# XuanchenLi/Topo4D

Hardware: AMD Instinct MI355X
Metric: rasterizer fwd+bwd views/sec (higher is better)
Workload: dtype f32

## Files before the change

### topo4d_amd/csrc/t4d_raster.hip

```cpp
#include <hip/hip_runtime.h>
#include <stdint.h>
#include <stdio.h>
#include <stdlib.h>
#include <string.h>
#include <vector>

#include "../../include/t4d_config.h"
#include "../../include/topo4d_raster.h"
#include "t4d_activations.h"

#define T4D_EXPORT extern "C" __attribute__((visibility("default")))

namespace {

constexpr int kBlock = 256;
#ifndef T4D_FWD_BATCH
#define T4D_FWD_BATCH 192
#endif
constexpr int kFwdBatch = T4D_FWD_BATCH;
#ifndef T4D_BWD_BATCH
#define T4D_BWD_BATCH 128
#endif
constexpr int kBwdBatch = T4D_BWD_BATCH;
constexpr int kSortLdsCap = 2048;
constexpr int kLongBlock = 1024;
constexpr int kScanChunk = 1024;
constexpr int kRankSortMax = 512;
constexpr int kHist = 1024;
constexpr int kBuckets = 24;
constexpr int kGP = T4D_GRAD_PAIR_FLOATS;
constexpr int kCursorSegs = 64;
#ifndef T4D_SEG
#define T4D_SEG 128
#endif
constexpr int kSeg = T4D_SEG;
constexpr int kSegOne = 64;
constexpr int kSegMaxTiles = 8192;
#ifndef T4D_SEG_LONG_MIN
#define T4D_SEG_LONG_MIN 2048
#endif
constexpr int kSegLongMin = T4D_SEG_LONG_MIN;
constexpr int kSnapFloats = 6;
static_assert((kSegLongMin & (kSegLongMin - 1)) == 0, "k_fwd_long_prefix stops at the first work item of a shorter length CLASS (powers of two)");

thread_local char g_err[512] = "";

enum KernelId { K_PREPROCESS = 0, K_SCAN_TILES, K_SCATTER, K_SORT_TILES, K_RENDER_FWD, K_RENDER_BWD, K_PREPROCESS_BWD,
                K_SORT_LONG, K_FWD_LONG, K_RENDER_BWD_LONG, K_COUNT };
const char *const kKernelNames[K_COUNT] = { "k_preprocess", "k_scan_tiles", "k_scatter", "k_sort_tiles", "k_render_fwd",
                                            "k_render_bwd", "k_preprocess_bwd", "k_sort_long", "k_fwd_long", "k_render_bwd_long" };
struct ProfRec { int id; hipEvent_t a, b; };
bool g_prof_on = false;
std::vector<ProfRec> g_prof;

struct Layout {
    size_t status, view_total, view_cursor, tile_count, bucket_fill, slot_tab, zero_end;
    size_t snap, live;
    size_t tile_off, chunk_sum, order, items, xy, depth, conic_opacity, rgb, clamped, pair_off, pair_rank, keys, sort_tmp, final_T, n_contrib, total;
};

struct DevStatus {
    uint32_t overflow;
    uint32_t max_pairs;
    unsigned long long total_pairs;
    uint32_t max_tile_pairs;
    uint32_t grid_sync;
    uint32_t live_segments;
};

inline size_t align_up(size_t x, size_t a = 256) { return (x + a - 1) / a * a; }

inline int seg_mode(const T4DProblem &p)
{
    const long long T = (long long)((p.W + T4D_TILE_X - 1) / T4D_TILE_X) * (long long)((p.H + T4D_TILE_Y - 1) / T4D_TILE_Y);
    if ((long long)p.n_views * T <= kSegMaxTiles) return 1;
    return p.n_views == 1 ? 2 : 0;
}
inline bool seg_capable(const T4DProblem &p) { return seg_mode(p) != 0; }
inline int seg_positions(const T4DProblem &p) { return (p.n_views == 1 && seg_mode(p) == 1) ? kSegOne : kSeg; }
inline size_t seg_slots_per_view(const T4DProblem &p, size_t T)
{
    if (seg_mode(p) == 2) return (size_t)p.pair_capacity / (size_t)kSeg + (size_t)p.pair_capacity / (size_t)kSegLongMin + 2;
    return (size_t)p.pair_capacity / (size_t)seg_positions(p) + T + 1;
}

Layout make_layout(const T4DProblem &p)
{
    Layout L;
    const size_t V = (size_t)p.n_views, P = (size_t)p.P;
    const size_t T = (size_t)((p.W + T4D_TILE_X - 1) / T4D_TILE_X) * (size_t)((p.H + T4D_TILE_Y - 1) / T4D_TILE_Y);
    const size_t HW = (size_t)p.H * p.W;
    const size_t cap = (size_t)p.pair_capacity;
    size_t o = 0;
    L.status = o;        o = align_up(o + sizeof(DevStatus));
    L.view_total = o;    o = align_up(o + V * 4);
    L.view_cursor = o;   o = align_up(o + V * kCursorSegs * 4);
    L.tile_count = o;    o = align_up(o + V * T * 4);
    L.bucket_fill = o;   o = align_up(o + kBuckets * 4);
    const size_t slots = seg_capable(p) ? V * seg_slots_per_view(p, T) : 0;
    L.slot_tab = o;      o = align_up(o + slots * 16);
    L.zero_end = o;
    L.snap = o;          o = align_up(o + slots * kSnapFloats * kBlock * 4);
    L.live = o;          o = align_up(o + (seg_mode(p) == 2 ? slots * 4 : 0));
    L.tile_off = o;      o = align_up(o + V * T * 4);
    L.chunk_sum = o;     o = align_up(o + V * ((T + kScanChunk - 1) / kScanChunk) * 4);
    L.order = o;         o = align_up(o + (size_t)kBuckets * V * T * 4);
    L.items = o;         o = align_up(o + V * T * 16);
    L.xy = o;            o = align_up(o + V * P * 8);
    L.depth = o;         o = align_up(o + V * P * 4);
    L.conic_opacity = o; o = align_up(o + V * P * 16);
    L.rgb = o;           o = align_up(o + (p.sh_coeffs > 0 ? V * P * 12 : 0));
    L.clamped = o;       o = align_up(o + (p.sh_coeffs > 0 ? V * P : 0));
    L.pair_off = o;      o = align_up(o + V * P * 4);
    L.pair_rank = o;     o = align_up(o + V * cap * 4);
    L.keys = o;          o = align_up(o + V * cap * 8);
    L.sort_tmp = o;      o = align_up(o + V * cap * 8);
    L.final_T = o;       o = align_up(o + V * HW * 4);
    L.n_contrib = o;     o = align_up(o + V * HW * 4);
    L.total = o;
    return L;
}

struct KP {
    int V, P, H, W, gx, gy, T, deg, M;
    float scale_modifier;
    uint32_t cap;
    uint32_t nseg, seg_cap;
    uint32_t seg_shift;
    const float *views, *means3D, *opacities, *scales, *rotations, *cov3D_precomp, *colors_precomp, *shs;
    DevStatus *status;
    uint32_t *view_total, *view_cursor, *tile_count, *bucket_fill, *tile_off, *chunk_sum, *order, *pair_off, *pair_rank;
    int n_chunks;
    int long_bins_elsewhere;
    int raw_params;
    uint4 *items;
    float2 *xy;
    float *depth;
    float4 *conic_opacity;
    float *rgb;
    uint8_t *clamped;
    unsigned long long *keys, *sort_tmp;
    float *cut_r2;
    float *final_T;
    uint32_t *n_contrib;
    float *out_color, *out_depth, *out_alpha;
    int32_t *radii;
    const float *dL_dcolor, *dL_ddepth, *dL_dalpha;
    float *grad_pair;
    float *dL_dmeans3D, *dL_dmeans2D, *dL_dcolors, *dL_dshs, *dL_dopacities, *dL_dscales, *dL_drotations, *dL_dcov3D;
    float *tile_dot;
    float *cotangent_dot;
    uint32_t tile_blocks;
    uint32_t fill_blocks;
    uint32_t fill_vec;
    uint4 *slot_tab;
    float *snap;
    uint32_t slots_per_view;
    uint32_t fused_sort;
    unsigned long long *host_status;
    uint32_t seg_min_pairs;
    uint32_t *live;
    uint32_t slots_by_offset;
    uint32_t views_per_set;
};

__device__ __forceinline__ float ndc2pix(float v, int S)
{
#pragma clang fp contract(off)
    return ((v + 1.0f) * S - 1.0f) * 0.5f;
}

__device__ __forceinline__ void tile_rect(float px, float py, int r, int gx, int gy, int &x0, int &y0, int &x1, int &y1)
{
    x0 = min(gx, max(0, (int)((px - r) / T4D_TILE_X)));
    y0 = min(gy, max(0, (int)((py - r) / T4D_TILE_Y)));
    x1 = min(gx, max(0, (int)((px + r + T4D_TILE_X - 1) / T4D_TILE_X)));
    y1 = min(gy, max(0, (int)((py + r + T4D_TILE_Y - 1) / T4D_TILE_Y)));
}

typedef const __attribute__((address_space(4))) float *const_float_p;
struct ViewRecord {
    float view[16], proj[16], campos[3], bg[3], tanx, tany;
};
__device__ __forceinline__ ViewRecord load_view_record(const float *views, const int v)
{
    const_float_p p = (const_float_p)(views + (size_t)v * T4D_VIEW_FLOATS);
    ViewRecord r;
#pragma unroll
    for (int i = 0; i < 16; i++) { r.view[i] = p[i]; r.proj[i] = p[16 + i]; }
#pragma unroll
    for (int i = 0; i < 3; i++) { r.campos[i] = p[32 + i]; r.bg[i] = p[35 + i]; }
    r.tanx = p[38]; r.tany = p[39];
    return r;
}

__device__ __forceinline__ size_t param_row0(const KP &kp, const int v)
{
    return kp.views_per_set ? (size_t)((uint32_t)v / kp.views_per_set) * (size_t)kp.P : (size_t)0;
}

__device__ __forceinline__ uint32_t seg_slot0(const KP &kp, const uint32_t off, const uint32_t tile)
{
    static_assert((kSegLongMin & (kSegLongMin - 1)) == 0, "a shift");
    return (off >> kp.seg_shift) + (kp.slots_by_offset ? off / (uint32_t)kSegLongMin : tile);
}

__device__ __forceinline__ uint32_t wave_incl_scan(uint32_t v)
{
    const int lane = threadIdx.x & 63;
#pragma unroll
    for (int d = 1; d < 64; d <<= 1) {
        uint32_t o = __shfl_up(v, d, 64);
        if (lane >= d) v += o;
    }
    return v;
}

template <int CTRL, int ROW_MASK = 0xf, int BANK_MASK = 0xf>
__device__ __forceinline__ float dpp0(float v)
{
    return __int_as_float(__builtin_amdgcn_update_dpp(0, __float_as_int(v), CTRL, ROW_MASK, BANK_MASK, false));
}

__device__ __forceinline__ float wave_sum_to_lane63(float v)
{
    v += dpp0<0xB1>(v);
    v += dpp0<0x4E>(v);
    v += dpp0<0x141>(v);
    v += dpp0<0x140>(v);
    v += dpp0<0x142, 0xA>(v);
    v += dpp0<0x143, 0xC>(v);
    return v;
}

__device__ __forceinline__ void quat_rot(const float4 q, float R[9])
{
#pragma clang fp contract(off)
    const float r = q.x, x = q.y, y = q.z, z = q.w;
    R[0] = 1.f - 2.f * (y * y + z * z); R[1] = 2.f * (x * y - r * z);       R[2] = 2.f * (x * z + r * y);
    R[3] = 2.f * (x * y + r * z);       R[4] = 1.f - 2.f * (x * x + z * z); R[5] = 2.f * (y * z - r * x);
    R[6] = 2.f * (x * z - r * y);       R[7] = 2.f * (y * z + r * x);       R[8] = 1.f - 2.f * (x * x + y * y);
}

__device__ __forceinline__ void cov3d_from_scale_rot(const float *scale, float mod, const float4 q, float cov[6])
{
#pragma clang fp contract(off)
// ... 149 lines not shown
        if (debug) {                                                                           \
            e_ = hipStreamSynchronize(stream);                                                 \
            if (e_ != hipSuccess) return fail(T4D_ERR_HIP, name " exec: %s", hipGetErrorString(e_)); \
        }                                                                                      \
    } while (0)

int device_cus()
{
    static int cus = 0;
    if (cus == 0) {
        int dev = 0, n = 0;
        if (hipGetDevice(&dev) != hipSuccess || hipDeviceGetAttribute(&n, hipDeviceAttributeMultiprocessorCount, dev) != hipSuccess || n <= 0)
            n = 256;
        cus = n;
    }
    return cus;
}

int tile_grid(int n_tiles, int per_cu, int div)
{
    static int env_div = -1;
    if (env_div < 0) {
        const char *d = getenv("T4D_TILE_DIV");
        env_div = d ? atoi(d) : 0;
    }
    if (env_div > 0) return max(min(n_tiles, device_cus() * per_cu), (n_tiles + env_div - 1) / env_div);
    constexpr int kMaxGridPerCu = 96;
    return max(min(n_tiles, device_cus() * per_cu), min((n_tiles + div - 1) / div, device_cus() * kMaxGridPerCu));
}

bool latency_launch(int n_tiles)
{
    const char *e = getenv("T4D_LATENCY_TILES");
    return n_tiles <= (e ? atoi(e) : 4 * device_cus());
}
bool latency_launch_fwd(int n_tiles, uint32_t flags)
{
    const char *e = getenv("T4D_FWD_LATENCY_TILES");
    if (!e) e = getenv("T4D_LATENCY_TILES");
    return n_tiles <= (e ? atoi(e) : ((flags & T4D_FLAG_LONG_LISTS) ? 24 : 12) * device_cus());
}

int check_problem(const T4DProblem *p)
{
    if (!p) return fail(T4D_ERR_ARG, "null problem");
    if (p->abi_version != T4D_ABI_VERSION) return fail(T4D_ERR_ARG, "abi_version mismatch");
    if (p->n_views < 1 || p->P < 1 || p->H < 1 || p->W < 1) return fail(T4D_ERR_ARG, "n_views, P, H, W must be >= 1");
    if (p->n_views > 4095) return fail(T4D_ERR_ARG, "n_views must be <= 4095");
    if ((int64_t)((p->W + T4D_TILE_X - 1) / T4D_TILE_X) * ((p->H + T4D_TILE_Y - 1) / T4D_TILE_Y) > 0xfffff)
        return fail(T4D_ERR_ARG, "image too large: more than 2^20 tiles");
    if ((int64_t)p->n_views * ((p->W + T4D_TILE_X - 1) / T4D_TILE_X) * ((p->H + T4D_TILE_Y - 1) / T4D_TILE_Y) > (1LL << 30))
        return fail(T4D_ERR_ARG, "n_views * tiles exceeds 2^30 work items: split the batch");
    if (p->pair_capacity < 1 || p->pair_capacity > 0x7fffffffLL) return fail(T4D_ERR_ARG, "pair_capacity out of range");
    if (p->views_per_param_set != 0u && (p->views_per_param_set > (uint32_t)p->n_views || (uint32_t)p->n_views % p->views_per_param_set != 0u))
        return fail(T4D_ERR_ARG, "n_views must be a multiple of views_per_param_set");
    if (p->sh_coeffs < 0 || p->sh_degree < 0 || p->sh_degree > 3) return fail(T4D_ERR_ARG, "sh_degree must be 0..3");
    if (p->sh_coeffs > 0 && p->sh_coeffs < (p->sh_degree + 1) * (p->sh_degree + 1))
        return fail(T4D_ERR_ARG, "sh_coeffs smaller than (sh_degree+1)^2");
    return T4D_OK;
}

void fill_common(KP &kp, const T4DProblem &p, const Layout &L, char *st)
{
    kp.V = p.n_views; kp.P = p.P; kp.H = p.H; kp.W = p.W;
    kp.gx = (p.W + T4D_TILE_X - 1) / T4D_TILE_X;
    kp.gy = (p.H + T4D_TILE_Y - 1) / T4D_TILE_Y;
    kp.T = kp.gx * kp.gy;
    kp.deg = p.sh_degree; kp.M = p.sh_coeffs;
    kp.scale_modifier = p.scale_modifier;
    kp.raw_params = (p.flags & T4D_FLAG_RAW_PARAMS) ? 1 : 0;
    kp.views_per_set = (p.views_per_param_set != 0u && p.views_per_param_set < (uint32_t)p.n_views) ? p.views_per_param_set : 0u;
    kp.cap = (uint32_t)p.pair_capacity;
    {
        const uint32_t n_wg = (uint32_t)((p.P + kBlock - 1) / kBlock);
        kp.nseg = 1;
        while (kp.nseg < (uint32_t)kCursorSegs && n_wg >= 16u * kp.nseg) kp.nseg <<= 1;
        kp.seg_cap = kp.cap / kp.nseg;
    }
    kp.status = reinterpret_cast<DevStatus *>(st + L.status);
    kp.view_total = reinterpret_cast<uint32_t *>(st + L.view_total);
    kp.view_cursor = reinterpret_cast<uint32_t *>(st + L.view_cursor);
    kp.tile_count = reinterpret_cast<uint32_t *>(st + L.tile_count);
    kp.bucket_fill = reinterpret_cast<uint32_t *>(st + L.bucket_fill);
    kp.order = reinterpret_cast<uint32_t *>(st + L.order);
    kp.items = reinterpret_cast<uint4 *>(st + L.items);
    kp.pair_rank = reinterpret_cast<uint32_t *>(st + L.pair_rank);
    kp.cut_r2 = reinterpret_cast<float *>(st + L.pair_rank);
    kp.tile_off = reinterpret_cast<uint32_t *>(st + L.tile_off);
    kp.chunk_sum = reinterpret_cast<uint32_t *>(st + L.chunk_sum);
    kp.n_chunks = (kp.T + kScanChunk - 1) / kScanChunk;
    kp.long_bins_elsewhere = (p.flags & T4D_FLAG_NO_LONG_BINS) ? 0 : 1;
    kp.pair_off = reinterpret_cast<uint32_t *>(st + L.pair_off);
    kp.xy = reinterpret_cast<float2 *>(st + L.xy);
    kp.depth = reinterpret_cast<float *>(st + L.depth);
    kp.conic_opacity = reinterpret_cast<float4 *>(st + L.conic_opacity);
    kp.rgb = reinterpret_cast<float *>(st + L.rgb);
    kp.clamped = reinterpret_cast<uint8_t *>(st + L.clamped);
    kp.keys = reinterpret_cast<unsigned long long *>(st + L.keys);
    kp.sort_tmp = reinterpret_cast<unsigned long long *>(st + L.sort_tmp);
    kp.final_T = reinterpret_cast<float *>(st + L.final_T);
    kp.n_contrib = reinterpret_cast<uint32_t *>(st + L.n_contrib);
    kp.slot_tab = reinterpret_cast<uint4 *>(st + L.slot_tab);
    kp.snap = reinterpret_cast<float *>(st + L.snap);
    kp.live = reinterpret_cast<uint32_t *>(st + L.live);
    kp.slots_per_view = seg_capable(p) ? (uint32_t)seg_slots_per_view(p, (size_t)kp.T) : 0u;
    kp.seg_shift = seg_positions(p) == 64 ? 6u : 7u;
    kp.slots_by_offset = seg_mode(p) == 2 ? 1u : 0u;
    kp.seg_min_pairs = seg_mode(p) == 2 ? ((p.flags & T4D_FLAG_NO_LONG_BINS) ? 0xffffffffu : (uint32_t)kSegLongMin) : 0u;
    static_assert(kSegOne == 64 && kSeg == 128, "seg_shift assumes segment lengths of 64 and 128");
}

}

T4D_EXPORT uint32_t t4d_abi_version(void) { return T4D_ABI_VERSION; }
T4D_EXPORT const char *t4d_last_error(void) { return g_err; }

T4D_EXPORT size_t t4d_state_bytes(const T4DProblem *prob)
{
    if (check_problem(prob) != T4D_OK) return 0;
    return make_layout(*prob).total;
}

size_t grad_pair_bytes(const T4DProblem &p) { return align_up((size_t)p.n_views * (size_t)p.pair_capacity * kGP * sizeof(float)); }
size_t tile_dot_bytes(const T4DProblem &p, size_t n_tiles) { return align_up((size_t)p.n_views * n_tiles * 4 * sizeof(float)); }

T4D_EXPORT size_t t4d_backward_scratch_bytes(const T4DProblem *prob)
{
    if (check_problem(prob) != T4D_OK) return 0;
    const size_t n_tiles = (size_t)((prob->W + T4D_TILE_X - 1) / T4D_TILE_X) * ((prob->H + T4D_TILE_Y - 1) / T4D_TILE_Y);
    return grad_pair_bytes(*prob) + tile_dot_bytes(*prob, n_tiles) +
           (prob->sh_coeffs > 0 ? align_up((size_t)prob->n_views * (size_t)prob->P * 3 * sizeof(float)) : 0);
}

T4D_EXPORT int t4d_debug_state_layout(const T4DProblem *prob, int has_sh, uint64_t *offsets, int n)
{
    int rc = check_problem(prob);
    if (rc != T4D_OK) return rc;
    if (!offsets || n < T4D_DEBUG_LAYOUT_FIELDS) return fail(T4D_ERR_ARG, "offsets must hold T4D_DEBUG_LAYOUT_FIELDS entries");
    T4DProblem p = *prob;
    if (!has_sh) p.sh_coeffs = 0;
    const Layout L = make_layout(p);
    const size_t f[T4D_DEBUG_LAYOUT_FIELDS] = { L.status, L.view_total, L.view_cursor, L.tile_count, L.bucket_fill, L.tile_off,
                                                L.xy, L.depth, L.conic_opacity, L.rgb, L.clamped, L.pair_off, L.keys,
                                                L.final_T, L.n_contrib, L.total };
    for (int i = 0; i < T4D_DEBUG_LAYOUT_FIELDS; i++) offsets[i] = (uint64_t)f[i];
    return T4D_OK;
}

static unsigned front_small_resident_blocks()
{
    static int cached_dev = -1;
    static unsigned cached = 0;
    int dev = 0;
    if (hipGetDevice(&dev) != hipSuccess) { (void)hipGetLastError(); return 0; }
    if (dev != cached_dev) {
        int per_cu = 0, cus = 0;
        if (hipOccupancyMaxActiveBlocksPerMultiprocessor(&per_cu, k_front_small, kBlock, 0) != hipSuccess ||
            hipDeviceGetAttribute(&cus, hipDeviceAttributeMultiprocessorCount, dev) != hipSuccess || per_cu < 1 || cus < 1) {
            (void)hipGetLastError();
            per_cu = 0; cus = 0;
        }
        cached = (unsigned)per_cu * (unsigned)cus;
        cached_dev = dev;
    }
    return cached;
}

T4D_EXPORT int t4d_rasterize_forward(const T4DProblem *prob, const T4DForwardIO *io, T4DStatus *status, void *hip_stream)
{
    int rc = check_problem(prob);
    if (rc != T4D_OK) return rc;
    if (!io || !io->views || !io->means3D || !io->opacities || !io->out_color || !io->out_depth || !io->out_alpha ||
        !io->out_radii || !io->state)
        return fail(T4D_ERR_ARG, "null required pointer in T4DForwardIO");
    if ((io->shs == nullptr) == (io->colors_precomp == nullptr))
        return fail(T4D_ERR_ARG, "provide exactly one of shs / colors_precomp");
    if (io->cov3D_precomp ? (io->scales || io->rotations) : (!io->scales || !io->rotations))
        return fail(T4D_ERR_ARG, "provide exactly one of (scales, rotations) / cov3D_precomp");
    if (io->shs && prob->sh_coeffs < 1) return fail(T4D_ERR_ARG, "shs given but sh_coeffs == 0");
    T4DProblem p = *prob;
    if (!io->shs) p.sh_coeffs = 0;
    const Layout L = make_layout(p);
    if (io->state_bytes < L.total) return fail(T4D_ERR_STATE_SIZE, "state buffer smaller than t4d_state_bytes()");
    hipStream_t stream = (hipStream_t)hip_stream;
    const bool debug = (p.flags & T4D_FLAG_DEBUG_SYNC) != 0;
    const bool checked = debug || (p.flags & T4D_FLAG_CHECKED) != 0;
    char *st = (char *)io->state;

    KP kp;
    memset(&kp, 0, sizeof(kp));
    fill_common(kp, p, L, st);
    kp.views = io->views; kp.means3D = io->means3D; kp.opacities = io->opacities; kp.scales = io->scales;
    kp.rotations = io->rotations; kp.cov3D_precomp = io->cov3D_precomp; kp.colors_precomp = io->colors_precomp;
    kp.shs = io->shs;
    kp.out_color = io->out_color; kp.out_depth = io->out_depth; kp.out_alpha = io->out_alpha; kp.radii = io->out_radii;

    bool status_published = false;
    if (!checked && (p.flags & T4D_FLAG_ASYNC_STATUS) && status && p.n_views == 1 && kp.T <= kSmallTiles &&
        getenv("T4D_NO_SMALL_VIEW") == nullptr && getenv("T4D_STATUS_BY_COPY") == nullptr) {
        void *dptr = nullptr;
        if (hipHostGetDevicePointer(&dptr, (void *)status, 0) == hipSuccess && dptr != nullptr) {
            kp.host_status = (unsigned long long *)dptr;
            status_published = true;
        } else {
            (void)hipGetLastError();
        }
    }
    T4D_HIP(hipMemsetAsync(st, 0, L.zero_end, stream));
    const bool small_view = p.n_views == 1 && kp.T <= kSmallTiles && getenv("T4D_NO_SMALL_VIEW") == nullptr;
    const bool front = small_view && gaussian_grid(p.P, 1) + 1u <= 128u && gaussian_grid(p.P, 1) + 1u <= front_small_resident_blocks() &&
                       getenv("T4D_NO_FRONT_FUSION") == nullptr;
    { ProfScope ps_(stream, K_PREPROCESS);
    if (front) hipLaunchKernelGGL(k_front_small, dim3(gaussian_grid(p.P, 1) + 1), dim3(kBlock), 0, stream, kp);
    else hipLaunchKernelGGL(k_preprocess, dim3(gaussian_grid(p.P, p.n_views)), dim3(kBlock), 0, stream, kp);
    }
    T4D_LAUNCH_CHECK("k_preprocess");
    if (front) {
    } else if (small_view) {
        ProfScope ps_(stream, K_SCATTER);
        hipLaunchKernelGGL(k_scan_scatter_small, dim3(gaussian_grid(p.P, 1) + 1), dim3(kBlock), 0, stream, kp);
    } else {
        ProfScope ps_(stream, K_SCAN_TILES);
        if (kp.n_chunks > 1) hipLaunchKernelGGL(k_tile_chunk_sums, dim3(kp.n_chunks, p.n_views), dim3(kScanChunk), 0, stream, kp);
        hipLaunchKernelGGL(k_scan_tiles, dim3(kp.n_chunks, p.n_views), dim3(kScanChunk), 0, stream, kp);
    }
    T4D_LAUNCH_CHECK("k_scan_tiles");
    if (checked) {
        DevStatus hs;
        T4D_HIP(hipMemcpyAsync(&hs, st + L.status, sizeof(hs), hipMemcpyDeviceToHost, stream));
        T4D_HIP(hipStreamSynchronize(stream));
        if (status) {
            status->max_pairs_per_view = hs.max_pairs;
            status->total_pairs = (int64_t)hs.total_pairs;
            status->overflow = (int32_t)hs.overflow;
            status->max_tile_pairs = (int32_t)min(hs.max_tile_pairs, 0x7fffffffu);
        }
        if (hs.overflow) return fail(T4D_ERR_PAIR_OVERFLOW, "pair_capacity too small for this scene");
    } else if ((p.flags & T4D_FLAG_ASYNC_STATUS) && status && !status_published) {
        T4D_HIP(hipMemcpyAsync((void *)status, st + L.status, 16, hipMemcpyDeviceToHost, stream));
    }
    if (!small_view) {
        ProfScope ps_(stream, K_SCATTER);
        hipLaunchKernelGGL(k_scatter, dim3(gaussian_grid(p.P, p.n_views) + (unsigned)(((size_t)kp.T * p.n_views + kBlock - 1) / kBlock)), dim3(kBlock), 0, stream, kp);
    }
    T4D_LAUNCH_CHECK("k_scatter");
    const bool lat = latency_launch_fwd(kp.T * p.n_views, p.flags);
    kp.fused_sort = (lat && (p.flags & T4D_FLAG_SHORT_BINS) != 0 && getenv("T4D_NO_FUSED_SORT") == nullptr) ? 1u : 0u;
    const bool long_fwd = kp.slots_per_view != 0u && kp.seg_min_pairs != 0xffffffffu && seg_mode(p) == 2 && !lat && getenv("T4D_NO_LONG_FWD") == nullptr;
    if (long_fwd && getenv("T4D_NO_FUSED_SORT") == nullptr) kp.fused_sort = 1u;
    if (!kp.fused_sort) {
        ProfScope ps_(stream, K_SORT_TILES);
        if (seg_mode(p) == 1 && (p.flags & T4D_FLAG_SHORT_BINS) == 0 && getenv("T4D_SORT_256") == nullptr)
            hipLaunchKernelGGL(k_sort_tiles<kLongBlock>, dim3(min(kp.T * p.n_views, 4 * device_cus())), dim3(kLongBlock), 0, stream, kp);
        else
            hipLaunchKernelGGL(k_sort_tiles<kBlock>, dim3(tile_grid(kp.T * p.n_views, 5, 2)), dim3(kBlock), 0, stream, kp);
    }
    T4D_LAUNCH_CHECK("k_sort_tiles");
    if (kp.long_bins_elsewhere) {
        ProfScope ps_(stream, K_SORT_LONG);
        hipLaunchKernelGGL(k_sort_long_chunks, dim3(min(kp.T * p.n_views, 2 * device_cus())), dim3(kLongBlock), 0, stream, kp);
        hipLaunchKernelGGL(k_merge_long, dim3(min(kp.T * p.n_views, 2 * device_cus())), dim3(kLongBlock), 0, stream, kp);
    }
    T4D_LAUNCH_CHECK("k_sort_long");
    {
    kp.tile_blocks = (uint32_t)(lat ? kp.T * p.n_views : tile_grid(kp.T * p.n_views, 6, 2));
    kp.fill_blocks = (uint32_t)(kp.gy * p.n_views);
    kp.fill_vec = (p.W % 4 == 0 && (((uintptr_t)io->out_color | (uintptr_t)io->out_depth | (uintptr_t)io->out_alpha) & 15u) == 0) ? 1u : 0u;
    if (getenv("T4D_FILL_SCALAR")) kp.fill_vec = 0u;
    const dim3 fgrid(kp.tile_blocks + kp.fill_blocks);
    const bool seg = kp.slots_per_view != 0u && kp.seg_min_pairs != 0xffffffffu;
    const bool seg_one = seg && seg_positions(p) == kSegOne;
    if (long_fwd) {
        { ProfScope ps_(stream, K_RENDER_FWD);
        hipLaunchKernelGGL((k_render_fwd<false, kFwdBatch, 0, true, true>), fgrid, dim3(kBlock), 0, stream, kp);
        }
        T4D_LAUNCH_CHECK("k_render_fwd");
        ProfScope psl_(stream, K_FWD_LONG);
        KP kl = kp;
        kl.tile_blocks = min(kp.slots_per_view, (uint32_t)(8 * device_cus()));
        hipLaunchKernelGGL(k_fwd_long_seg<false>, dim3(kl.tile_blocks), dim3(kBlock), 0, stream, kl);
        T4D_LAUNCH_CHECK("k_fwd_long_seg");
        hipLaunchKernelGGL(k_fwd_long_prefix, dim3(min((uint32_t)kp.T, (uint32_t)(4 * device_cus()))), dim3(kBlock), 0, stream, kl);
        T4D_LAUNCH_CHECK("k_fwd_long_prefix");
        hipLaunchKernelGGL(k_fwd_long_seg<true>, dim3(kl.tile_blocks), dim3(kBlock), 0, stream, kl);
    } else {
    ProfScope ps_(stream, K_RENDER_FWD);
    if (lat) {
        if (seg_one) hipLaunchKernelGGL((k_render_fwd<true, kBlock, kSegOne, true>), fgrid, dim3(kBlock), 0, stream, kp);
        else if (seg) hipLaunchKernelGGL((k_render_fwd<true, kBlock, kSeg, true>), fgrid, dim3(kBlock), 0, stream, kp);
        else hipLaunchKernelGGL((k_render_fwd<true, kBlock, 0, true>), fgrid, dim3(kBlock), 0, stream, kp);
    } else if (seg_one) {
        hipLaunchKernelGGL((k_render_fwd<false, kBlock, kSegOne, true>), fgrid, dim3(kBlock), 0, stream, kp);
    } else if (seg) {
        hipLaunchKernelGGL((k_render_fwd<false, kBlock, kSeg, true>), fgrid, dim3(kBlock), 0, stream, kp);
    } else if (kp.long_bins_elsewhere && getenv("T4D_NO_PRUNE") == nullptr) {
        hipLaunchKernelGGL((k_render_fwd<false, kFwdBatch, 0, true>), fgrid, dim3(kBlock), 0, stream, kp);
    } else {
        hipLaunchKernelGGL((k_render_fwd<false, kFwdBatch, 0, false>), fgrid, dim3(kBlock), 0, stream, kp);
    }
    }
// ... 174 lines not shown
```

### topo4d_amd/csrc/t4d_raster_binning.h

```cpp
struct PreOut {
    uint32_t tiles, pbase;
    int x0, y0, x1, y1;
    float depth;
    bool fits;
};

__device__ __forceinline__ void preprocess_body(const KP &kp, const uint32_t gb, const uint32_t vb, PreOut &po)
{
#pragma clang fp contract(off)
    __shared__ uint32_t s_wave_tot[4];
    __shared__ uint32_t s_base;
    __shared__ int s_bb[4];
    __shared__ uint32_t s_hist[kHist], s_hbase[kHist];
    const int tid = threadIdx.x;
    const int g = (int)gb * kBlock + tid;
    const int v = (int)vb;
    po.tiles = 0; po.pbase = 0; po.x0 = po.y0 = po.x1 = po.y1 = 0; po.depth = 0.f; po.fits = false;
    const ViewRecord vrec = load_view_record(kp.views, v);
    const float *view = vrec.view, *proj = vrec.proj;
    const size_t vg = (size_t)v * kp.P + g;
    const size_t gp = param_row0(kp, v) + (size_t)g;

    uint32_t tiles = 0;
    int x0 = 0, y0 = 0, x1 = 0, y1 = 0;
    if (g < kp.P) {
        const float mean[3] = { kp.means3D[3 * gp], kp.means3D[3 * gp + 1], kp.means3D[3 * gp + 2] };
        float cov3_in[6] = { 0.f, 0.f, 0.f, 0.f, 0.f, 0.f }, sc[3] = { 0.f, 0.f, 0.f };
        float4 q = make_float4(1.f, 0.f, 0.f, 0.f);
        if (kp.cov3D_precomp) {
#pragma unroll
            for (int k = 0; k < 6; k++) cov3_in[k] = kp.cov3D_precomp[6 * gp + k];
        } else {
            sc[0] = kp.scales[3 * gp]; sc[1] = kp.scales[3 * gp + 1]; sc[2] = kp.scales[3 * gp + 2];
            q = reinterpret_cast<const float4 *>(kp.rotations)[gp];
        }
        float opacity = kp.opacities[gp];
        if (kp.raw_params) {
            opacity = t4d_act_sigmoid(opacity);
            if (!kp.cov3D_precomp) {
                sc[0] = t4d_act_exp(sc[0]); sc[1] = t4d_act_exp(sc[1]); sc[2] = t4d_act_exp(sc[2]);
                q = t4d_act_normalize(q);
            }
        }
        int radius = 0;
        const float pvz = view[2] * mean[0] + view[6] * mean[1] + view[10] * mean[2] + view[14];
        if (pvz > T4D_NEAR_CULL_Z) {
            const float hx = proj[0] * mean[0] + proj[4] * mean[1] + proj[8] * mean[2] + proj[12];
            const float hy = proj[1] * mean[0] + proj[5] * mean[1] + proj[9] * mean[2] + proj[13];
            const float hw = proj[3] * mean[0] + proj[7] * mean[1] + proj[11] * mean[2] + proj[15];
            const float pw = 1.0f / (hw + T4D_HOM_W_EPS);
            float cov3[6];
            if (kp.cov3D_precomp) {
#pragma unroll
                for (int k = 0; k < 6; k++) cov3[k] = cov3_in[k];
            } else {
                cov3d_from_scale_rot(sc, kp.scale_modifier, q, cov3);
            }
            const float tanx = vrec.tanx, tany = vrec.tany;
            const float fx = kp.W / (2.0f * tanx), fy = kp.H / (2.0f * tany);
            float T0[3], T1[3], t[3];
            bool inx, iny;
            ewa_rows(mean, view, fx, fy, tanx, tany, T0, T1, t, inx, iny);
            float v0[3], v1[3];
            sym3_mul(cov3, T0, v0);
            sym3_mul(cov3, T1, v1);
            const float a = T0[0] * v0[0] + T0[1] * v0[1] + T0[2] * v0[2] + T4D_COV2D_DILATION;
            const float b = T0[0] * v1[0] + T0[1] * v1[1] + T0[2] * v1[2];
            const float c = T1[0] * v1[0] + T1[1] * v1[1] + T1[2] * v1[2] + T4D_COV2D_DILATION;
            const float det = a * c - b * b;
            if (det != 0.0f) {
                const float det_inv = 1.f / det;
                const float mid = 0.5f * (a + c);
                const float l1 = mid + sqrtf(fmaxf(T4D_EIGEN_FLOOR, mid * mid - det));
                const float l2 = mid - sqrtf(fmaxf(T4D_EIGEN_FLOOR, mid * mid - det));
                const float my_radius = ceilf(T4D_RADIUS_SIGMAS * sqrtf(fmaxf(l1, l2)));
                const float px = ndc2pix(hx * pw, kp.W), py = ndc2pix(hy * pw, kp.H);
                tile_rect(px, py, (int)my_radius, kp.gx, kp.gy, x0, y0, x1, y1);
                tiles = (uint32_t)((x1 - x0) * (y1 - y0));
                if (tiles > 0) {
                    radius = (int)my_radius;
                    po.depth = pvz;
                    kp.xy[vg] = make_float2(px, py);
                    kp.depth[vg] = pvz;
                    kp.conic_opacity[vg] = make_float4(c * det_inv, -b * det_inv, a * det_inv, opacity);
                    if (kp.shs) {
                        float d[3] = { mean[0] - vrec.campos[0], mean[1] - vrec.campos[1], mean[2] - vrec.campos[2] };
                        const float len = sqrtf(d[0] * d[0] + d[1] * d[1] + d[2] * d[2]);
                        d[0] /= len; d[1] /= len; d[2] /= len;
                        float bas[16];
// ... 17 lines not shown
                        uint32_t cl = 0;
#pragma unroll
                        for (int ch = 0; ch < 3; ch++) {
                            float r = 0.f;
#pragma unroll
                            for (int k = 0; k < 16; k++)
                                if (k < K) r += bas[k] * shl[k * 3 + ch];
                            r += 0.5f;
                            if (r < 0.f) cl |= 1u << ch;
                            kp.rgb[vg * 3 + ch] = fmaxf(r, 0.f);
                        }
                        kp.clamped[vg] = (uint8_t)cl;
                    }
                }
            }
        }
        kp.radii[vg] = radius;
    }

    const uint32_t incl = wave_incl_scan(tiles);
    const int wave = tid >> 6, lane = tid & 63;
    if (lane == 63) s_wave_tot[wave] = incl;
    if (tid == 0) { s_bb[0] = 0x7fffffff; s_bb[1] = 0x7fffffff; s_bb[2] = 0; s_bb[3] = 0; }
    __syncthreads();
    uint32_t wave_off = 0, block_tot = 0;
#pragma unroll
    for (int w = 0; w < 4; w++) {
        const uint32_t t = s_wave_tot[w];
        if (w < wave) wave_off += t;
        block_tot += t;
    }
    if (block_tot == 0) {
        if (g < kp.P) kp.pair_off[vg] = 0;
        return;
    }
    const uint32_t seg = gb & (kp.nseg - 1u);
    if (tid == 0) s_base = seg * kp.seg_cap + atomicAdd(&kp.view_cursor[v * kCursorSegs + seg], block_tot);
    {
        int bx0 = tiles ? x0 : 0x7fffffff, by0 = tiles ? y0 : 0x7fffffff, bx1 = tiles ? x1 : 0, by1 = tiles ? y1 : 0;
#pragma unroll
        for (int d = 32; d > 0; d >>= 1) {
            bx0 = min(bx0, __shfl_xor(bx0, d, 64)); by0 = min(by0, __shfl_xor(by0, d, 64));
            bx1 = max(bx1, __shfl_xor(bx1, d, 64)); by1 = max(by1, __shfl_xor(by1, d, 64));
        }
        if (lane == 0) { atomicMin(&s_bb[0], bx0); atomicMin(&s_bb[1], by0); atomicMax(&s_bb[2], bx1); atomicMax(&s_bb[3], by1); }
    }
    __syncthreads();
    const uint32_t pbase = s_base + wave_off + incl - tiles;
    const bool fits = pbase + tiles <= (seg + 1u) * kp.seg_cap;
    if (g < kp.P) kp.pair_off[vg] = fits ? pbase : kp.cap;
    po.tiles = tiles; po.pbase = pbase; po.x0 = x0; po.y0 = y0; po.x1 = x1; po.y1 = y1; po.fits = fits;

    uint32_t *cnt = kp.tile_count + (size_t)v * kp.T;
    uint32_t *prank = kp.pair_rank + (size_t)v * kp.cap;
    const int bbx = s_bb[0], bby = s_bb[1], bw = s_bb[2] - s_bb[0], bh = s_bb[3] - s_bb[1];
    const int area = bw * bh;
    if (area <= kHist) {
        for (int i = tid; i < area; i += kBlock) s_hist[i] = 0;
        __syncthreads();
        for (int y = y0; y < y1; y++)
            for (int x = x0; x < x1; x++) atomicAdd(&s_hist[(y - bby) * bw + (x - bbx)], 1u);
        __syncthreads();
        for (int i = tid; i < area; i += kBlock) {
            const uint32_t c = s_hist[i];
            const int ty = i / bw, tx = i - ty * bw;
            s_hbase[i] = c ? atomicAdd(&cnt[(bby + ty) * kp.gx + bbx + tx], c) : 0u;
            s_hist[i] = 0;
        }
        __syncthreads();
        uint32_t pr = pbase;
        for (int y = y0; y < y1; y++)
            for (int x = x0; x < x1; x++, pr++) {
                const int i = (y - bby) * bw + (x - bbx);
                const uint32_t r = s_hbase[i] + atomicAdd(&s_hist[i], 1u);
                if (fits) prank[pr] = r;
            }
    } else {
        uint32_t pr = pbase;
        for (int y = y0; y < y1; y++)
            for (int x = x0; x < x1; x++, pr++) {
                const uint32_t r = atomicAdd(&cnt[y * kp.gx + x], 1u);
                if (fits) prank[pr] = r;
            }
    }
}

__global__ __launch_bounds__(kBlock) void k_preprocess(const KP kp)
{
    const uint32_t nblocks = (uint32_t)(kp.P + kBlock - 1) / kBlock;
    uint32_t gb, vb;
    vb = blockIdx.x / nblocks; gb = blockIdx.x - vb * nblocks;
    if (vb >= (uint32_t)kp.V) return;
    PreOut po;
    preprocess_body(kp, gb, vb, po);
}

__device__ __forceinline__ int count_bucket(const uint32_t c)
{
    if (c == 0) return kBuckets - 1;
    return (kBuckets - 2) - min(kBuckets - 2, 31 - __clz((int)c));
}

struct TileOrder {
    uint32_t pre[kBuckets + 1];
};

__device__ __forceinline__ void load_tile_order(const KP &kp, TileOrder &o)
{
    uint32_t acc = 0;
#pragma unroll
    for (int k = 0; k < kBuckets; k++) {
        o.pre[k] = acc;
        acc += kp.bucket_fill[k];
    }
    o.pre[kBuckets] = acc;
}

__device__ __forceinline__ uint32_t tile_order_id(const KP &kp, const TileOrder &o, const uint32_t b)
{
    int k = 0;
    uint32_t base = 0;
#pragma unroll
    for (int i = 1; i < kBuckets; i++)
        if (b >= o.pre[i]) { k = i; base = o.pre[i]; }
    return kp.order[(size_t)k * kp.V * kp.T + (b - base)];
}

__global__ __launch_bounds__(kScanChunk) void k_tile_chunk_sums(const KP kp)
{
    __shared__ uint32_t s_w[kScanChunk / 64];
    const int v = blockIdx.y, c = blockIdx.x, tid = threadIdx.x, t = c * kScanChunk + tid;
    uint32_t x = t < kp.T ? kp.tile_count[(size_t)v * kp.T + t] : 0u;
#pragma unroll
    for (int d = 32; d > 0; d >>= 1) x += (uint32_t)__shfl_xor((int)x, d, 64);
    if ((tid & 63) == 0) s_w[tid >> 6] = x;
    __syncthreads();
    if (tid == 0) {
        uint32_t tot = 0;
#pragma unroll
        for (int w = 0; w < kScanChunk / 64; w++) tot += s_w[w];
        kp.chunk_sum[(size_t)v * kp.n_chunks + c] = tot;
    }
}

__global__ __launch_bounds__(kScanChunk) void k_scan_tiles(const KP kp)
{
    __shared__ uint32_t s_wave_tot[16], s_wave_max[16];
    __shared__ uint32_t s_carry;
    __shared__ uint32_t s_bcnt[kBuckets], s_bbase[kBuckets];
    const int v = blockIdx.y, chunk = blockIdx.x, tid = threadIdx.x, wave = tid >> 6, lane = tid & 63;
    const uint32_t *cnt = kp.tile_count + (size_t)v * kp.T;
    uint32_t *off = kp.tile_off + (size_t)v * kp.T;
    if (chunk == 0) {
        if (tid == 0) s_carry = 0;
    } else if (wave == 0) {
        uint32_t part = 0;
        for (int i = lane; i < chunk; i += 64) part += kp.chunk_sum[(size_t)v * kp.n_chunks + i];
#pragma unroll
        for (int d = 32; d > 0; d >>= 1) part += (uint32_t)__shfl_xor((int)part, d, 64);
        if (lane == 0) s_carry = part;
    }
    if (tid < kBuckets) s_bcnt[tid] = 0;
    __syncthreads();
    const int t = chunk * kScanChunk + tid;
    const uint32_t c = t < kp.T ? cnt[t] : 0u;
    const uint32_t incl = wave_incl_scan(c);
    uint32_t longest = c;
#pragma unroll
    for (int d = 32; d > 0; d >>= 1) longest = max(longest, (uint32_t)__shfl_xor((int)longest, d, 64));
    if (lane == 63) { s_wave_tot[wave] = incl; s_wave_max[wave] = longest; }
    const int bk = count_bucket(c);
    uint32_t r = 0;
    if (t < kp.T) r = atomicAdd(&s_bcnt[bk], 1u);
    __syncthreads();
    uint32_t woff = 0, tot = 0;
    longest = 0;
#pragma unroll
    for (int w = 0; w < 16; w++) {
        const uint32_t x = s_wave_tot[w];
        if (w < wave) woff += x;
        tot += x;
        longest = max(longest, s_wave_max[w]);
    }
    const uint32_t carry = s_carry;
    if (t < kp.T) off[t] = carry + woff + incl - c;
    if (tid < kBuckets) s_bbase[tid] = s_bcnt[tid] ? atomicAdd(&kp.bucket_fill[tid], s_bcnt[tid]) : 0u;
    if (tid == 0 && longest > 0) atomicMax(&kp.status->max_tile_pairs, longest);
    __syncthreads();
    if (t < kp.T) kp.order[(size_t)bk * kp.V * kp.T + s_bbase[bk] + r] = ((uint32_t)v << 20) | (uint32_t)t;
    if (tid == 0 && chunk == kp.n_chunks - 1) {
        const uint32_t total = carry + tot;
        kp.view_total[v] = total;
        uint32_t fill = 0;
        for (uint32_t k = 0; k < kp.nseg; k++) fill = max(fill, kp.view_cursor[v * kCursorSegs + k]);
        const unsigned long long need = max((unsigned long long)total, (unsigned long long)fill * kp.nseg);
        atomicMax(&kp.status->max_pairs, (uint32_t)min(need, 0xffffffffull));
        atomicAdd(&kp.status->total_pairs, (unsigned long long)total);
        if (total > kp.cap || fill > kp.seg_cap) atomicOr(&kp.status->overflow, 1u);
    }
}

template <bool BIG>
__device__ __forceinline__ void write_segment_slots(const KP &kp, const uint32_t id, const uint32_t off, const uint32_t n)
{
    if (kp.slots_per_view == 0u || n == 0u) return;
    if (BIG && n < kp.seg_min_pairs) return;
    const uint32_t nseg = (n + (1u << kp.seg_shift) - 1u) >> kp.seg_shift;
    const size_t first = (size_t)(id >> 20) * kp.slots_per_view + seg_slot0(kp, off, id & 0xfffffu);
    uint4 *tab = kp.slot_tab + first;
    for (uint32_t j = 0; j < nseg; j++) tab[j] = make_uint4(id, off, n, j | 0x80000000u);
    if (BIG && kp.slots_by_offset) {
        const uint32_t at = atomicAdd(&kp.status->live_segments, nseg);
        for (uint32_t j = 0; j < nseg; j++) kp.live[at + j] = (uint32_t)first + j;
    }
}

__global__ __launch_bounds__(kBlock) void k_scatter(const KP kp)
{
    const uint32_t nb8 = gaussian_grid(kp.P, 1);
    const uint32_t n_scatter = nb8 * (uint32_t)kp.V;
    if (blockIdx.x >= n_scatter) {
        const uint32_t b = (blockIdx.x - n_scatter) * kBlock + threadIdx.x;
        if (b >= (uint32_t)(kp.V * kp.T)) return;
        TileOrder ord;
        load_tile_order(kp, ord);
        const uint32_t id = tile_order_id(kp, ord, b);
        const size_t vt = (size_t)(id >> 20) * kp.T + (id & 0xfffffu);
        const uint32_t off = kp.tile_off[vt];
        const uint32_t n = off >= kp.cap ? 0u : min(kp.tile_count[vt], kp.cap - off);
        kp.items[b] = make_uint4(id, off, n, kp.tile_count[vt]);
        write_segment_slots<true>(kp, id, off, n);
        return;
    }
    const int v = (int)(blockIdx.x / nb8);
    const int g = (int)(blockIdx.x - (uint32_t)v * nb8) * kBlock + threadIdx.x;
    if (g >= kp.P) return;
    const size_t vg = (size_t)v * kp.P + g;
    const int r = kp.radii[vg];
    const float2 p = kp.xy[vg];
    const float dep = kp.depth[vg];
    uint32_t pr = kp.pair_off[vg];
    if (r <= 0) return;
    int x0, y0, x1, y1;
    tile_rect(p.x, p.y, r, kp.gx, kp.gy, x0, y0, x1, y1);
    const unsigned long long key = ((unsigned long long)__float_as_uint(dep) << 32) | (uint32_t)g;
    const uint32_t *off = kp.tile_off + (size_t)v * kp.T;
    const uint32_t *prank = kp.pair_rank + (size_t)v * kp.cap;
    unsigned long long *keys = kp.keys + (size_t)v * kp.cap;
    for (int y = y0; y < y1; y++)
        for (int x = x0; x < x1; x++, pr++) {
            if (pr >= kp.cap) return;
            const uint32_t pos = off[y * kp.gx + x] + prank[pr];
            if (pos < kp.cap) keys[pos] = key;
        }
}

constexpr int kSmallTiles = 4 * kBlock;

__device__ __forceinline__ void publish_status(const KP &kp, const uint32_t overflow, const uint32_t max_pairs, const unsigned long long total)
{
    if (kp.host_status == nullptr) return;
    __hip_atomic_store(&kp.host_status[1], total, __ATOMIC_RELAXED, __HIP_MEMORY_SCOPE_SYSTEM);
    __hip_atomic_store(&kp.host_status[0], (unsigned long long)overflow | ((unsigned long long)max_pairs << 32), __ATOMIC_RELEASE, __HIP_MEMORY_SCOPE_SYSTEM);
}

__global__ __launch_bounds__(kBlock) void k_scan_scatter_small(const KP kp)
{
    __shared__ uint32_t s_off[kSmallTiles];
    __shared__ uint32_t s_wtot[4];
    __shared__ uint32_t s_bcnt[kBuckets], s_bpre[kBuckets];
    __shared__ uint32_t s_longest[4];
    const int tid = threadIdx.x, wave = tid >> 6, lane = tid & 63;
    uint32_t c[4];
#pragma unroll
    for (int j = 0; j < 4; j++) c[j] = 4 * tid + j < kp.T ? kp.tile_count[4 * tid + j] : 0u;
    const uint32_t mine = (c[0] + c[1]) + (c[2] + c[3]);
    const uint32_t incl = wave_incl_scan(mine);
    if (lane == 63) s_wtot[wave] = incl;
    if (tid < kBuckets) s_bcnt[tid] = 0;
    __syncthreads();
    uint32_t base = incl - mine, total = 0;
#pragma unroll
    for (int w = 0; w < 4; w++) {
        const uint32_t x = s_wtot[w];
        if (w < wave) base += x;
        total += x;
    }
    uint32_t off[4];
    off[0] = base; off[1] = off[0] + c[0]; off[2] = off[1] + c[1]; off[3] = off[2] + c[2];
#pragma unroll
    for (int j = 0; j < 4; j++) s_off[4 * tid + j] = off[j];
    const uint32_t nb8 = gaussian_grid(kp.P, 1);
    if (blockIdx.x == nb8) {
        uint32_t longest = max(max(c[0], c[1]), max(c[2], c[3]));
#pragma unroll
        for (int d = 32; d > 0; d >>= 1) longest = max(longest, (uint32_t)__shfl_xor((int)longest, d, 64));
        if (lane == 0) s_longest[wave] = longest;
        int bk[4];
        uint32_t rank[4];
#pragma unroll
        for (int j = 0; j < 4; j++) {
            bk[j] = count_bucket(c[j]);
            rank[j] = 4 * tid + j < kp.T ? atomicAdd(&s_bcnt[bk[j]], 1u) : 0u;
        }
        __syncthreads();
        if (tid == 0) {
            uint32_t acc = 0;
            for (int k = 0; k < kBuckets; k++) { s_bpre[k] = acc; acc += s_bcnt[k]; }
        }
        __syncthreads();
        if (tid < kBuckets) kp.bucket_fill[tid] = s_bcnt[tid];
#pragma unroll
        for (int j = 0; j < 4; j++) {
            const int t = 4 * tid + j;
            if (t < kp.T) {
                kp.tile_off[t] = off[j];
                const uint32_t n = off[j] >= kp.cap ? 0u : min(c[j], kp.cap - off[j]);
                kp.items[s_bpre[bk[j]] + rank[j]] = make_uint4((uint32_t)t, off[j], n, c[j]);
                write_segment_slots<false>(kp, (uint32_t)t, off[j], n);
            }
        }
        if (tid == 0) {
            kp.view_total[0] = total;
            uint32_t fill = 0;
            for (uint32_t k = 0; k < kp.nseg; k++) fill = max(fill, kp.view_cursor[k]);
            const unsigned long long need = max((unsigned long long)total, (unsigned long long)fill * kp.nseg);
            kp.status->max_pairs = (uint32_t)min(need, 0xffffffffull);
            kp.status->total_pairs = (unsigned long long)total;
            kp.status->max_tile_pairs = max(max(s_longest[0], s_longest[1]), max(s_longest[2], s_longest[3]));
            const uint32_t ovf = (total > kp.cap || fill > kp.seg_cap) ? 1u : 0u;
            if (ovf) kp.status->overflow = 1u;
            publish_status(kp, ovf, (uint32_t)min(need, 0xffffffffull), (unsigned long long)total);
        }
        return;
    }
    __syncthreads();
    const int g = (int)blockIdx.x * kBlock + tid;
    if (g >= kp.P) return;
    const int r = kp.radii[g];
    const float2 p = kp.xy[g];
    const float dep = kp.depth[g];
    uint32_t pr = kp.pair_off[g];
    if (r <= 0) return;
    int x0, y0, x1, y1;
    tile_rect(p.x, p.y, r, kp.gx, kp.gy, x0, y0, x1, y1);
    const unsigned long long key = ((unsigned long long)__float_as_uint(dep) << 32) | (uint32_t)g;
    for (int y = y0; y < y1; y++)
        for (int x = x0; x < x1; x++, pr++) {
            if (pr >= kp.cap) return;
            const uint32_t pos = s_off[y * kp.gx + x] + kp.pair_rank[pr];
            if (pos < kp.cap) kp.keys[pos] = key;
        }
}

__device__ __forceinline__ uint32_t load_agent(const uint32_t *p) { return __hip_atomic_load(p, __ATOMIC_RELAXED, __HIP_MEMORY_SCOPE_AGENT); }

__global__ __launch_bounds__(kBlock) void k_front_small(const KP kp)
{
    __shared__ uint32_t s_off[kSmallTiles];
    __shared__ uint32_t s_wtot[4];
    __shared__ uint32_t s_bcnt[kBuckets], s_bpre[kBuckets];
    __shared__ uint32_t s_longest[4];
    const int tid = threadIdx.x, wave = tid >> 6, lane = tid & 63;
    const uint32_t nb8 = gaussian_grid(kp.P, 1), nblocks = (uint32_t)(kp.P + kBlock - 1) / kBlock;
    PreOut po;
    po.tiles = 0; po.pbase = 0; po.x0 = po.y0 = po.x1 = po.y1 = 0; po.depth = 0.f; po.fits = false;
    if (blockIdx.x < nblocks) preprocess_body(kp, blockIdx.x, 0u, po);
    __syncthreads();
    if (tid == 0) {
        __hip_atomic_fetch_add(&kp.status->grid_sync, 1u, __ATOMIC_RELAXED, __HIP_MEMORY_SCOPE_AGENT);
        while (load_agent(&kp.status->grid_sync) < nb8 + 1u) __builtin_amdgcn_s_sleep(2);
    }
    __syncthreads();
    uint32_t c[4];
#pragma unroll
    for (int j = 0; j < 4; j++) c[j] = 4 * tid + j < kp.T ? load_agent(&kp.tile_count[4 * tid + j]) : 0u;
    const uint32_t mine = (c[0] + c[1]) + (c[2] + c[3]);
    const uint32_t incl = wave_incl_scan(mine);
    if (lane == 63) s_wtot[wave] = incl;
    if (tid < kBuckets) s_bcnt[tid] = 0;
    __syncthreads();
    uint32_t base = incl - mine, total = 0;
#pragma unroll
    for (int w = 0; w < 4; w++) {
        const uint32_t x = s_wtot[w];
        if (w < wave) base += x;
        total += x;
    }
    uint32_t off[4];
    off[0] = base; off[1] = off[0] + c[0]; off[2] = off[1] + c[1]; off[3] = off[2] + c[2];
#pragma unroll
    for (int j = 0; j < 4; j++) s_off[4 * tid + j] = off[j];
    if (blockIdx.x == nb8) {
        uint32_t longest = max(max(c[0], c[1]), max(c[2], c[3]));
#pragma unroll
        for (int d = 32; d > 0; d >>= 1) longest = max(longest, (uint32_t)__shfl_xor((int)longest, d, 64));
        if (lane == 0) s_longest[wave] = longest;
        int bk[4];
        uint32_t rank[4];
#pragma unroll
        for (int j = 0; j < 4; j++) {
            bk[j] = count_bucket(c[j]);
            rank[j] = 4 * tid + j < kp.T ? atomicAdd(&s_bcnt[bk[j]], 1u) : 0u;
        }
        __syncthreads();
        if (tid == 0) {
            uint32_t acc = 0;
            for (int k = 0; k < kBuckets; k++) { s_bpre[k] = acc; acc += s_bcnt[k]; }
        }
        __syncthreads();
        if (tid < kBuckets) kp.bucket_fill[tid] = s_bcnt[tid];
#pragma unroll
        for (int j = 0; j < 4; j++) {
            const int t = 4 * tid + j;
            if (t < kp.T) {
                kp.tile_off[t] = off[j];
                const uint32_t n = off[j] >= kp.cap ? 0u : min(c[j], kp.cap - off[j]);
                kp.items[s_bpre[bk[j]] + rank[j]] = make_uint4((uint32_t)t, off[j], n, c[j]);
                write_segment_slots<false>(kp, (uint32_t)t, off[j], n);
            }
        }
        if (tid == 0) {
            kp.view_total[0] = total;
            uint32_t fill = 0;
            for (uint32_t k = 0; k < kp.nseg; k++) fill = max(fill, load_agent(&kp.view_cursor[k]));
            const unsigned long long need = max((unsigned long long)total, (unsigned long long)fill * kp.nseg);
            kp.status->max_pairs = (uint32_t)min(need, 0xffffffffull);
            kp.status->total_pairs = (unsigned long long)total;
            kp.status->max_tile_pairs = max(max(s_longest[0], s_longest[1]), max(s_longest[2], s_longest[3]));
            const uint32_t ovf = (total > kp.cap || fill > kp.seg_cap) ? 1u : 0u;
            if (ovf) kp.status->overflow = 1u;
            publish_status(kp, ovf, (uint32_t)min(need, 0xffffffffull), (unsigned long long)total);
        }
        return;
    }
    __syncthreads();
    if (po.tiles == 0u || !po.fits) return;
    const int g = (int)blockIdx.x * kBlock + tid;
    const unsigned long long key = ((unsigned long long)__float_as_uint(po.depth) << 32) | (uint32_t)g;
// ... 10 lines not shown
```

Before: 56330.

## Fuse per-view tile scan into preprocess via last-block ticket

Adds a per-view ticket counter so the last preprocess block to finish for a view performs the tile-count prefix scan and bucket ordering inline, removing the separate scan kernel launch when a view fits in one scan chunk. The ticket is hierarchical over cursor segments and relies on a waitcnt plus relaxed agent-scope atomics for visibility. This cuts one launch and its dependency gap, but serializes the scan onto one block at the tail and depends on correct memory ordering.

```diff
diff --git a/topo4d_amd/csrc/t4d_raster.hip b/topo4d_amd/csrc/t4d_raster.hip
--- a/topo4d_amd/csrc/t4d_raster.hip
+++ b/topo4d_amd/csrc/t4d_raster.hip
@@ -54,7 +54,7 @@
 std::vector<ProfRec> g_prof;
 
 struct Layout {
-    size_t status, view_total, view_cursor, tile_count, bucket_fill, slot_tab, zero_end;
+    size_t status, view_total, view_cursor, tile_count, bucket_fill, scan_ticket, slot_tab, zero_end;
     size_t snap, live;
     size_t tile_off, chunk_sum, order, items, xy, depth, conic_opacity, rgb, clamped, pair_off, pair_rank, keys, sort_tmp, final_T, n_contrib, total;
 };
@@ -97,6 +97,7 @@
     L.view_cursor = o;   o = align_up(o + V * kCursorSegs * 4);
     L.tile_count = o;    o = align_up(o + V * T * 4);
     L.bucket_fill = o;   o = align_up(o + kBuckets * 4);
+    L.scan_ticket = o;   o = align_up(o + V * (kCursorSegs + 1) * 4);
     const size_t slots = seg_capable(p) ? V * seg_slots_per_view(p, T) : 0;
     L.slot_tab = o;      o = align_up(o + slots * 16);
     L.zero_end = o;
@@ -162,6 +163,7 @@
     uint32_t *live;
     uint32_t slots_by_offset;
     uint32_t views_per_set;
+    uint32_t *scan_ticket;
 };
 
 __device__ __forceinline__ float ndc2pix(float v, int S)
@@ -477,6 +479,7 @@
     kp.view_cursor = reinterpret_cast<uint32_t *>(st + L.view_cursor);
     kp.tile_count = reinterpret_cast<uint32_t *>(st + L.tile_count);
     kp.bucket_fill = reinterpret_cast<uint32_t *>(st + L.bucket_fill);
+    kp.scan_ticket = reinterpret_cast<uint32_t *>(st + L.scan_ticket);
     kp.order = reinterpret_cast<uint32_t *>(st + L.order);
     kp.items = reinterpret_cast<uint4 *>(st + L.items);
     kp.pair_rank = reinterpret_cast<uint32_t *>(st + L.pair_rank);
@@ -605,12 +608,14 @@
     const bool small_view = p.n_views == 1 && kp.T <= kSmallTiles && getenv("T4D_NO_SMALL_VIEW") == nullptr;
     const bool front = small_view && gaussian_grid(p.P, 1) + 1u <= 128u && gaussian_grid(p.P, 1) + 1u <= front_small_resident_blocks() &&
                        getenv("T4D_NO_FRONT_FUSION") == nullptr;
+    const bool pre_scan = seg_mode(p) == 0 && kp.n_chunks == 1 && getenv("T4D_NO_PREPROCESS_SCAN") == nullptr;
     { ProfScope ps_(stream, K_PREPROCESS);
     if (front) hipLaunchKernelGGL(k_front_small, dim3(gaussian_grid(p.P, 1) + 1), dim3(kBlock), 0, stream, kp);
-    else hipLaunchKernelGGL(k_preprocess, dim3(gaussian_grid(p.P, p.n_views)), dim3(kBlock), 0, stream, kp);
+    else if (pre_scan) hipLaunchKernelGGL(k_preprocess<true>, dim3(gaussian_grid(p.P, p.n_views)), dim3(kBlock), 0, stream, kp);
+    else hipLaunchKernelGGL(k_preprocess<false>, dim3(gaussian_grid(p.P, p.n_views)), dim3(kBlock), 0, stream, kp);
     }
     T4D_LAUNCH_CHECK("k_preprocess");
-    if (front) {
+    if (front || pre_scan) {
     } else if (small_view) {
         ProfScope ps_(stream, K_SCATTER);
         hipLaunchKernelGGL(k_scan_scatter_small, dim3(gaussian_grid(p.P, 1) + 1), dim3(kBlock), 0, stream, kp);
diff --git a/topo4d_amd/csrc/t4d_raster_binning.h b/topo4d_amd/csrc/t4d_raster_binning.h
--- a/topo4d_amd/csrc/t4d_raster_binning.h
+++ b/topo4d_amd/csrc/t4d_raster_binning.h
@@ -5,6 +5,7 @@
     bool fits;
 };
 
+template <bool SCAN = false>
 __device__ __forceinline__ void preprocess_body(const KP &kp, const uint32_t gb, const uint32_t vb, PreOut &po)
 {
 #pragma clang fp contract(off)
@@ -188,17 +189,8 @@
                 const uint32_t r = atomicAdd(&cnt[y * kp.gx + x], 1u);
                 if (fits) prank[pr] = r;
             }
-    }
-}
-
-__global__ __launch_bounds__(kBlock) void k_preprocess(const KP kp)
-{
-    const uint32_t nblocks = (uint32_t)(kp.P + kBlock - 1) / kBlock;
-    uint32_t gb, vb;
-    vb = blockIdx.x / nblocks; gb = blockIdx.x - vb * nblocks;
-    if (vb >= (uint32_t)kp.V) return;
-    PreOut po;
-    preprocess_body(kp, gb, vb, po);
+        if (SCAN) __builtin_amdgcn_s_waitcnt(0);
+    }
 }
 
 __device__ __forceinline__ int count_bucket(const uint32_t c)
@@ -303,6 +295,91 @@
         atomicMax(&kp.status->max_pairs, (uint32_t)min(need, 0xffffffffull));
         atomicAdd(&kp.status->total_pairs, (unsigned long long)total);
         if (total > kp.cap || fill > kp.seg_cap) atomicOr(&kp.status->overflow, 1u);
+    }
+}
+
+__device__ __forceinline__ uint32_t load_agent(const uint32_t *p) { return __hip_atomic_load(p, __ATOMIC_RELAXED, __HIP_MEMORY_SCOPE_AGENT); }
+
+__device__ __forceinline__ void scan_view_tiles(const KP &kp, const int v)
+{
+    __shared__ uint32_t s_wtot[4], s_wmax[4];
+    __shared__ uint32_t s_bcnt[kBuckets], s_bbase[kBuckets];
+    const int tid = threadIdx.x, wave = tid >> 6, lane = tid & 63;
+    const uint32_t *cnt = kp.tile_count + (size_t)v * kp.T;
+    uint32_t *off = kp.tile_off + (size_t)v * kp.T;
+    if (tid < kBuckets) s_bcnt[tid] = 0;
+    uint32_t c[4];
+#pragma unroll
+    for (int j = 0; j < 4; j++) c[j] = 4 * tid + j < kp.T ? load_agent(&cnt[4 * tid + j]) : 0u;
+    const uint32_t mine = (c[0] + c[1]) + (c[2] + c[3]);
+    const uint32_t incl = wave_incl_scan(mine);
+    uint32_t longest = max(max(c[0], c[1]), max(c[2], c[3]));
+#pragma unroll
+    for (int d = 32; d > 0; d >>= 1) longest = max(longest, (uint32_t)__shfl_xor((int)longest, d, 64));
+    if (lane == 63) { s_wtot[wave] = incl; s_wmax[wave] = longest; }
+    __syncthreads();
+    int bk[4];
+    uint32_t rank[4];
+#pragma unroll
+    for (int j = 0; j < 4; j++) {
+        bk[j] = count_bucket(c[j]);
+        rank[j] = 4 * tid + j < kp.T ? atomicAdd(&s_bcnt[bk[j]], 1u) : 0u;
+    }
+    uint32_t base = incl - mine, total = 0;
+    longest = 0;
+#pragma unroll
+    for (int w = 0; w < 4; w++) {
+        const uint32_t x = s_wtot[w];
+        if (w < wave) base += x;
+        total += x;
+        longest = max(longest, s_wmax[w]);
+    }
+#pragma unroll
+    for (int j = 0; j < 4; j++) {
+        if (4 * tid + j < kp.T) off[4 * tid + j] = base;
+        base += c[j];
+    }
+    __syncthreads();
+    if (tid < kBuckets) s_bbase[tid] = s_bcnt[tid] ? atomicAdd(&kp.bucket_fill[tid], s_bcnt[tid]) : 0u;
+    if (tid == 0 && longest > 0) atomicMax(&kp.status->max_tile_pairs, longest);
+    __syncthreads();
+#pragma unroll
+    for (int j = 0; j < 4; j++) {
+        const int t = 4 * tid + j;
+        if (t < kp.T) kp.order[(size_t)bk[j] * kp.V * kp.T + s_bbase[bk[j]] + rank[j]] = ((uint32_t)v << 20) | (uint32_t)t;
+    }
+    if (tid == 0) {
+        kp.view_total[v] = total;
+        uint32_t fill = 0;
+        for (uint32_t k = 0; k < kp.nseg; k++) fill = max(fill, load_agent(&kp.view_cursor[v * kCursorSegs + k]));
+        const unsigned long long need = max((unsigned long long)total, (unsigned long long)fill * kp.nseg);
+        atomicMax(&kp.status->max_pairs, (uint32_t)min(need, 0xffffffffull));
+        atomicAdd(&kp.status->total_pairs, (unsigned long long)total);
+        if (total > kp.cap || fill > kp.seg_cap) atomicOr(&kp.status->overflow, 1u);
+    }
+}
+
+template <bool SCAN>
+__global__ __launch_bounds__(kBlock) void k_preprocess(const KP kp)
+{
+    const uint32_t nblocks = (uint32_t)(kp.P + kBlock - 1) / kBlock;
+    uint32_t gb, vb;
+    vb = blockIdx.x / nblocks; gb = blockIdx.x - vb * nblocks;
+    if (vb >= (uint32_t)kp.V) return;
+    PreOut po;
+    preprocess_body<SCAN>(kp, gb, vb, po);
+    if (SCAN) {
+        __shared__ uint32_t s_last;
+        __syncthreads();
+        if (threadIdx.x == 0) {
+            const uint32_t seg = gb & (kp.nseg - 1u), in_seg = (nblocks - seg + kp.nseg - 1u) / kp.nseg;
+            uint32_t *tk = kp.scan_ticket + (size_t)vb * (kCursorSegs + 1);
+            bool last = __hip_atomic_fetch_add(&tk[1 + seg], 1u, __ATOMIC_RELAXED, __HIP_MEMORY_SCOPE_AGENT) == in_seg - 1u;
+            if (last) last = __hip_atomic_fetch_add(&tk[0], 1u, __ATOMIC_RELAXED, __HIP_MEMORY_SCOPE_AGENT) == kp.nseg - 1u;
+            s_last = last;
+        }
+        __syncthreads();
+        if (s_last) scan_view_tiles(kp, (int)vb);
     }
 }
 
@@ -459,8 +536,6 @@
         }
 }
 
-__device__ __forceinline__ uint32_t load_agent(const uint32_t *p) { return __hip_atomic_load(p, __ATOMIC_RELAXED, __HIP_MEMORY_SCOPE_AGENT); }
-
 __global__ __launch_bounds__(kBlock) void k_front_small(const KP kp)
 {
     __shared__ uint32_t s_off[kSmallTiles];
```

Result: no change. 56160 (median of 2 runs) (-0.3%).
